# nullmax-vision/SimPB

Hardware: AMD Instinct MI355X
Metric: frames/sec (6-cam sample) + MSDeformAttn HBM GB/s, R50 704x256 @1/2/4/8 GPU (higher is better)
Workload: dtype f32

## Files before the change

include/simpb_hip.h:

```cpp
#ifndef SIMPB_HIP_H
#define SIMPB_HIP_H

#ifdef __cplusplus
extern "C" {
#endif

#define SIMPB_OK 0
#define SIMPB_EINVAL 1
#define SIMPB_ELAUNCH 2

#define SIMPB_RECORD3D_WIDTH 15

int simpb_abi_version(void);

const char* simpb_last_error(void);

#define SIMPB_KERNEL_DAF 1
#define SIMPB_KERNEL_MSDA 2
int simpb_timing_enable(int capacity);
int simpb_timing_read(int kernel_id, float* ms_out, int max_n);
void simpb_timing_reset(void);

int simpb_deformable_aggregation_forward(
    float* output, const float* mc_ms_feat, const int* spatial_shape, const int* scale_start_index,
// ... 276 lines not shown
                           int num_anchors, int num_cams, int num_levels, int num_pts, int num_groups,
                           const unsigned char* cam_valid, void* stream);

int simpb_alloc_project(unsigned char* flag, float* sel_xy, float* depth, const float* anchor,
                        const float* projection_mat, int batch_size, int num_anchors, int num_cams,
                        float img_w, float img_h, float limit_w, float limit_l, float limit_h, void* stream);
int simpb_alloc_project_cams(unsigned char* flag, float* sel_xy, float* depth, const float* anchor,
                             const float* projection_mat, int batch_size, int num_anchors, int num_cams, float img_w,
                             float img_h, float limit_w, float limit_l, float limit_h, const unsigned char* cam_valid,
                             void* stream);

int simpb_alloc_compact(int* count, int* order, const unsigned char* flag, int batch_size, int num_anchors,
                        int num_cams, void* stream);

int simpb_alloc_group_start(int* group_start, int* overflow, const int* count, int batch_size, int num_cams,
                            int capacity, void* stream);

int simpb_alloc_scatter(float* ref_pts2d, float* ref_depth2d, int* q2a, int* is_center, int* a2q, int* query_cam,
                        const int* group_start, const int* count, const int* order, const unsigned char* flag,
                        const float* sel_xy, const float* depth, int batch_size, int num_anchors, int num_cams,
                        int num_query, float img_w, float img_h, void* stream);

int simpb_alloc_static(unsigned char* flag, float* sel_xy, float* depth, int* count, int* order, int* group_start,
                       int* overflow, float* ref_pts2d, float* ref_depth2d, int* q2a, int* is_center, int* a2q,
                       int* query_cam, const float* anchor, const float* projection_mat, int batch_size, int num_anchors,
                       int num_cams, int capacity, float img_w, float img_h, float limit_w, float limit_l, float limit_h,
                       void* stream);
int simpb_alloc_static_cams(unsigned char* flag, float* sel_xy, float* depth, int* count, int* order, int* group_start,
                            int* overflow, float* ref_pts2d, float* ref_depth2d, int* q2a, int* is_center, int* a2q,
                            int* query_cam, const float* anchor, const float* projection_mat, int batch_size,
                            int num_anchors, int num_cams, int capacity, float img_w, float img_h, float limit_w,
                            float limit_l, float limit_h, const unsigned char* cam_valid, void* stream);

int simpb_alloc_ragged(unsigned char* flag, float* sel_xy, float* depth, int* count, int* order, int* group_start,
                       int* overflow, float* ref_pts2d, float* ref_depth2d, int* q2a, int* is_center, int* a2q,
                       int* query_cam, const float* anchor, const float* projection_mat, int batch_size, int num_anchors,
                       int num_cams, int per_stream, float img_w, float img_h, float limit_w, float limit_l, float limit_h,
                       void* stream);
int simpb_alloc_ragged_active(unsigned char* flag, float* sel_xy, float* depth, int* count, int* order, int* group_start,
                              int* overflow, float* ref_pts2d, float* ref_depth2d, int* q2a, int* is_center, int* a2q,
                              int* query_cam, const float* anchor, const float* projection_mat, int batch_size,
                              int num_anchors, int num_cams, int per_stream, float img_w, float img_h, float limit_w,
                              float limit_l, float limit_h, const unsigned char* active, void* stream);
int simpb_alloc_ragged_cams(unsigned char* flag, float* sel_xy, float* depth, int* count, int* order, int* group_start,
                            int* overflow, float* ref_pts2d, float* ref_depth2d, int* q2a, int* is_center, int* a2q,
                            int* query_cam, const float* anchor, const float* projection_mat, int batch_size,
                            int num_anchors, int num_cams, int per_stream, float img_w, float img_h, float limit_w,
                            float limit_l, float limit_h, const unsigned char* active, const unsigned char* cam_valid,
                            void* stream);

int simpb_gather_rows(float* out, const float* src, const int* q2a, int batch_size, int num_anchors,
                      int num_query, int channels, void* stream);

int simpb_aggregate_2d_to_3d(float* out_q, float* out_pos, const float* q3d, const float* pos3d, const float* q2d,
                             const float* pos2d, const float* alpha, const int* a2q, int batch_size,
                             int num_anchors, int num_cams, int num_query, int channels, void* stream);

int simpb_aggregate_2d_to_3d_alpha(float* out_q, float* out_pos, const float* q3d, const float* pos3d, const float* q2d,
                                   const float* pos2d, const float* alpha, const int* a2q, const float* hidden,
                                   int ld_hidden, int hidden_dim, const float* w_alpha, const float* b_alpha,
                                   int batch_size, int num_anchors, int num_cams, int num_query, int channels,
                                   void* stream);

#ifdef __cplusplus
}
#endif
// ... 2 lines not shown
```

simpb_amd/_lib.py:

```python
import ctypes
import os

from .build import LIB

_lib = None

_P = ctypes.c_void_p
_I = ctypes.c_int
_F = ctypes.c_float
_LL = ctypes.c_longlong


class WorldTables(ctypes.Structure):
    _fields_ = [("class_range", _F * 32), ("attr_moving", ctypes.c_ubyte * 32), ("attr_still", ctypes.c_ubyte * 32),
                ("threshold", _F), ("has_threshold", _I), ("num_output", _I)]


SIGNATURES = {
    "simpb_abi_version": ([], _I),
    "simpb_last_error": ([], ctypes.c_char_p),
    "simpb_timing_enable": ([_I], _I),
    "simpb_timing_read": ([_I, _P, _I], _I),
    "simpb_timing_reset": ([], None),
    "simpb_deformable_aggregation_forward": ([_P] * 6 + [_I] * 8 + [_P], _I),
# ... 24 lines not shown
    "simpb_attention_f32_split": ([_P] * 6 + [_I] * 9 + [_F, _P], _I),
    "simpb_attention_split_halfs": ([_P] * 6 + [_I] * 9 + [_P], _I),
    "simpb_mlp_chain_forward": ([_P, _P], _I),
    "simpb_bank_get": ([_P] * 6 + [_I] * 2 + [_F] * 2 + [_P], _I),
    "simpb_bank_update": ([_P] * 10 + [_I] * 5 + [_P], _I),
    "simpb_bank_update_rank": ([_P, _P] + [_I] * 4 + [_P], _I),
    "simpb_bank_update_merge": ([_P] * 13 + [_I, _P] + [_I] * 5 + [_P], _I),
    "simpb_bank_update_merge_active": ([_P] * 13 + [_I, _P] + [_I] * 5 + [_P, _P], _I),
    "simpb_bank_cache": ([_P] * 10 + [_I] * 6 + [_F, _I, _F, _P, _I, _P, _P], _I),
    "simpb_bank_cache_streams": ([_P] * 10 + [_I] * 6 + [_F, _I, _F, _P, _I, _P, _P, _P], _I),
    "simpb_bank_cache_streams_active": ([_P] * 10 + [_I] * 6 + [_F, _I, _F, _P, _I, _P, _P, _P, _P], _I),
    "simpb_decode3d_record": ([_P] * 6 + [_I] * 4 + [_P], _I),
    "simpb_decode2d_record": ([_P] * 6 + [_I] * 4 + [_F] * 4 + [_P], _I),
    "simpb_record2d_compact": ([_P, _LL, _P, _LL, _I, _I, _I, _P], _I),
    "simpb_decode2d_record_ragged": ([_P] * 7 + [_I] * 5 + [_F] * 4 + [_P], _I),
    "simpb_world_record": ([_P] * 5 + [WorldTables, _I, _P], _I),
    "simpb_topk_rows": ([_P, _P, _P, _I, _I, _I, _P], _I),
    "simpb_rowdot_sigmoid": ([_P, _P, _I, _P, _P, _I, _I, _P, _P], _I),
    "simpb_anchor_projection": ([_P] * 4 + [_I] * 2 + [_P], _I),
    "simpb_msda_prep": ([_P, _P, _P, _I, _P, _I, _P, _I, _I, _I, _I, _P, _P], _I),
    "simpb_dfa_points": ([_P] * 7 + [_I] * 5 + [_P], _I),
    "simpb_dfa_weights": ([_P] * 3 + [_I] * 6 + [_P], _I),
    "simpb_dfa_points_cams": ([_P] * 7 + [_I] * 5 + [_P, _P], _I),
    "simpb_dfa_weights_cams": ([_P] * 3 + [_I] * 6 + [_P, _P], _I),
    "simpb_alloc_project_cams": ([_P] * 5 + [_I] * 3 + [_F] * 5 + [_P, _P], _I),
    "simpb_alloc_project": ([_P] * 5 + [_I] * 3 + [_F] * 5 + [_P], _I),
    "simpb_alloc_compact": ([_P] * 3 + [_I] * 3 + [_P], _I),
    "simpb_alloc_group_start": ([_P] * 3 + [_I] * 3 + [_P], _I),
    "simpb_alloc_scatter": ([_P] * 12 + [_I] * 4 + [_F] * 2 + [_P], _I),
    "simpb_alloc_static": ([_P] * 15 + [_I] * 4 + [_F] * 5 + [_P], _I),
    "simpb_alloc_ragged": ([_P] * 15 + [_I] * 4 + [_F] * 5 + [_P], _I),
    "simpb_alloc_ragged_active": ([_P] * 15 + [_I] * 4 + [_F] * 5 + [_P, _P], _I),
    "simpb_alloc_static_cams": ([_P] * 15 + [_I] * 4 + [_F] * 5 + [_P, _P], _I),
    "simpb_alloc_ragged_cams": ([_P] * 15 + [_I] * 4 + [_F] * 5 + [_P, _P, _P], _I),
    "simpb_gather_rows": ([_P] * 3 + [_I] * 4 + [_P], _I),
    "simpb_aggregate_2d_to_3d": ([_P] * 8 + [_I] * 5 + [_P], _I),
    "simpb_aggregate_2d_to_3d_alpha": ([_P] * 9 + [_I, _I, _P, _P] + [_I] * 5 + [_P], _I),
}

ERRORS = {1: "SIMPB_EINVAL (bad pointer/size/layout)", 2: "SIMPB_ELAUNCH (kernel launch failed)"}


def lib():
    global _lib
    if _lib is None:
        if not os.path.exists(LIB):
            raise RuntimeError(
                f"{LIB} is missing: build it with `python -m simpb_amd.build` (hipcc --offload-arch=gfx950). "
                "simpb_amd has no fallback path for its HIP kernels.")
        import torch
        handle = ctypes.CDLL(LIB)
        for name, (argtypes, restype) in SIGNATURES.items():
            fn = getattr(handle, name)
            fn.argtypes = argtypes
            fn.restype = restype
        _lib = handle
    return _lib


def check(status, what):
    if status != 0:
        detail = ""
        if status == 2:
            detail = " - " + (lib().simpb_last_error() or b"").decode()
        raise RuntimeError(f"{what} failed: {ERRORS.get(status, status)}{detail}")
```

simpb_amd/csrc/alloc.hip:

```cpp
#include <hip/hip_runtime.h>
#include "../../include/simpb_hip.h"
#include "store_fence.h"

extern "C" int simpb_check_launch(void);

namespace {

constexpr int kMaxStaticCams = 8;

template <bool MASKED>
__global__ void alloc_project_kernel(unsigned char* __restrict__ flag, float* __restrict__ sel_xy,
                                     float* __restrict__ depth, const float* __restrict__ anchor,
                                     const float* __restrict__ proj, int bs, int A, int cams, float img_w, float img_h,
                                     float lim_w, float lim_l, float lim_h, int* __restrict__ a2q_fill,
                                     const unsigned char* __restrict__ active,
                                     const unsigned char* __restrict__ cam_valid) {
  const int idx = blockIdx.x * blockDim.x + threadIdx.x;
  if (idx >= bs * A * cams) return;
  const int cam = idx % cams;
  const int a = (idx / cams) % A;
  const int b = idx / (cams * A);
  bool off = active && !active[b];
  if (MASKED) off = off || !cam_valid[b * cams + cam];
  if (off) {
    const size_t o = ((size_t)b * cams + cam) * A + a;
    flag[o] = 0;
    sel_xy[2 * o] = 0.f;
    sel_xy[2 * o + 1] = 0.f;
    depth[o] = 0.f;
    if (a2q_fill) a2q_fill[idx] = -1;
    return;
  }
  const float* an = anchor + ((size_t)b * A + a) * 11;
  const float* P = proj + ((size_t)b * cams + cam) * 16;
  const float cx = an[0], cy = an[1], cz = an[2];
  const float sw = fminf(expf(an[3]), lim_w), sl = fminf(expf(an[4]), lim_l), sh = fminf(expf(an[5]), lim_h);
  const float sn = an[6], cs = an[7];

  float xmin = INFINITY, xmax = -INFINITY, ymin = INFINITY, ymax = -INFINITY;
  bool corner_valid = false;
  float ctr_x = 0.f, ctr_y = 0.f, ctr_d = 0.f;
  for (int k = 0; k < 9; ++k) {
    float px, py, pz;
    if (k < 8) {
      const float ox = (((k >> 2) & 1) - 0.5f) * sw, oy = (((k >> 1) & 1) - 0.5f) * sl, oz = ((k & 1) - 0.5f) * sh;
      px = cs * ox - sn * oy + cx;
      py = sn * ox + cs * oy + cy;
      pz = oz + cz;
    } else {
      px = cx; py = cy; pz = cz;
    }
    const float u = P[0] * px + P[1] * py + P[2] * pz + P[3];
    const float v = P[4] * px + P[5] * py + P[6] * pz + P[7];
    const float d = P[8] * px + P[9] * py + P[10] * pz + P[11];
    const float dc = fmaxf(d, 1e-5f);
    const float x = u / dc, y = v / dc;
    const bool inside = 0.f < x && x < img_w && 0.f < y && y < img_h;
    if (k < 8) {
      corner_valid = corner_valid || (d > 0.f && inside);
      xmin = fminf(xmin, x); xmax = fmaxf(xmax, x);
      ymin = fminf(ymin, y); ymax = fmaxf(ymax, y);
    } else {
      ctr_x = x; ctr_y = y; ctr_d = d;
    }
  }
  const bool center_valid = 0.f < ctr_x && ctr_x < img_w && 0.f < ctr_y && ctr_y < img_h;
  float sx = (fminf(fmaxf(xmin, 0.f), img_w) + fminf(fmaxf(xmax, 0.f), img_w)) / 2.f;
  float sy = (fminf(fmaxf(ymin, 0.f), img_h) + fminf(fmaxf(ymax, 0.f), img_h)) / 2.f;
  if (center_valid) { sx = ctr_x; sy = ctr_y; }
  const size_t o = ((size_t)b * cams + cam) * A + a;
  flag[o] = center_valid ? 2 : (corner_valid ? 1 : 0);
  sel_xy[2 * o] = sx;
  sel_xy[2 * o + 1] = sy;
  depth[o] = ctr_d;
  if (a2q_fill) a2q_fill[idx] = -1;
}

__global__ __launch_bounds__(256) void alloc_compact_kernel(int* __restrict__ count, int* __restrict__ order,
                                                            const unsigned char* __restrict__ flag, int A) {
  __shared__ int s_wave[4];
  __shared__ int s_base;
  const int bc = blockIdx.x;
  const unsigned char* f = flag + (size_t)bc * A;
  int* ord = order + (size_t)bc * A;
  const int lane = threadIdx.x & 63, wave = threadIdx.x >> 6;
  if (threadIdx.x == 0) s_base = 0;
  __syncthreads();
  for (int a0 = 0; a0 < A; a0 += 256) {
    const int a = a0 + threadIdx.x;
    const bool on = a < A && f[a] != 0;
    const unsigned long long m = __ballot(on);
    if (lane == 0) s_wave[wave] = __popcll(m);
    __syncthreads();
    int off = s_base;
    for (int w = 0; w < wave; ++w) off += s_wave[w];
    if (on) ord[off + __popcll(m & ((1ull << lane) - 1ull))] = a;
    __syncthreads();
    if (threadIdx.x == 0) s_base += s_wave[0] + s_wave[1] + s_wave[2] + s_wave[3];
    __syncthreads();
  }
  if (threadIdx.x == 0) count[bc] = s_base;
}

__global__ void alloc_scatter_kernel(float* __restrict__ ref_pts2d, float* __restrict__ ref_depth2d,
// ... 124 lines not shown
  is_center[slot] = ctr;
}

__global__ void alloc_group_start_kernel(int* __restrict__ group_start, int* __restrict__ overflow,
                                         const int* __restrict__ count, int bs, int cams, int capacity) {
  if (threadIdx.x != 0 || blockIdx.x != 0) return;
  int acc = 0;
  group_start[0] = 0;
  bool over = false;
  for (int c = 0; c < cams; ++c) {
    int m = 0;
    for (int b = 0; b < bs; ++b) m = max(m, count[b * cams + c]);
    acc += m;
    if (acc > capacity) { over = true; acc = capacity; }
    group_start[c + 1] = acc;
  }
  overflow[0] = over ? 1 : 0;
}

__global__ void fill_int_kernel(int* __restrict__ p, int v, size_t n) {
  const size_t i = (size_t)blockIdx.x * blockDim.x + threadIdx.x;
  if (i < n) p[i] = v;
}

__global__ void gather_rows_kernel(float* __restrict__ out, const float* __restrict__ src,
                                   const int* __restrict__ q2a, int A, int N2, int C4) {
  const int s = blockIdx.x, b = blockIdx.y;
  const int a = q2a[(size_t)b * N2 + s];
  float4* o = reinterpret_cast<float4*>(out) + ((size_t)b * N2 + s) * C4;
  const float4* r = reinterpret_cast<const float4*>(src) + ((size_t)b * A + max(a, 0)) * C4;
  for (int c = threadIdx.x; c < C4; c += blockDim.x) o[c] = a >= 0 ? r[c] : make_float4(0.f, 0.f, 0.f, 0.f);
}

constexpr int kMaxAggCams = 8;
__global__ __launch_bounds__(64) void aggregate_kernel(float* __restrict__ out_q, float* __restrict__ out_pos,
                                                       const float* __restrict__ q3d, const float* __restrict__ pos3d,
                                                       const float* __restrict__ q2d, const float* __restrict__ pos2d,
                                                       const float* __restrict__ alpha, const int* __restrict__ a2q, int A,
                                                       int cams, int N2, int C4, const float* __restrict__ hidden, int ldh,
                                                       int kh, const float* __restrict__ w_alpha,
                                                       const float* __restrict__ b_alpha) {
  const int a = blockIdx.x, b = blockIdx.y;
  const int* slots = a2q + ((size_t)b * A + a) * cams;
  float wgt[kMaxAggCams];
  int slot[kMaxAggCams];
  float div = 0.f;
#pragma unroll
  for (int k = 0; k < kMaxAggCams; ++k) {
    slot[k] = k < cams ? slots[k] : -1;
    wgt[k] = 0.f;
  }
#pragma unroll
  for (int k = 0; k < kMaxAggCams; ++k) {
    const int s = slot[k];
    if (s < 0) continue;
    float w;
    if (hidden) {
      const float* h = hidden + ((size_t)b * N2 + s) * ldh;
      float d = 0.f;
      for (int c = threadIdx.x * 4; c < kh; c += 256) {
        const float4 xv = *reinterpret_cast<const float4*>(h + c);
        const float4 wv = *reinterpret_cast<const float4*>(w_alpha + c);
        d += xv.x * wv.x + xv.y * wv.y + xv.z * wv.z + xv.w * wv.w;
      }
#pragma unroll
      for (int m = 32; m >= 1; m >>= 1) d += __shfl_xor(d, m);
// ... 140 lines not shown
                     out_q, out_pos, q3d, pos3d, q2d, pos2d, alpha, a2q, num_anchors, num_cams, num_query, channels / 4,
                     hidden, ld_hidden, hidden_dim, w_alpha, b_alpha);
  return status();
}

extern "C" int simpb_aggregate_2d_to_3d(float* out_q, float* out_pos, const float* q3d, const float* pos3d,
                                        const float* q2d, const float* pos2d, const float* alpha, const int* a2q,
                                        int batch_size, int num_anchors, int num_cams, int num_query, int channels,
                                        void* stream) {
  if (!alpha) return SIMPB_EINVAL;
  return simpb_aggregate_2d_to_3d_alpha(out_q, out_pos, q3d, pos3d, q2d, pos2d, alpha, a2q, nullptr, 0, 0, nullptr, nullptr,
                                        batch_size, num_anchors, num_cams, num_query, channels, stream);
}

extern "C" int simpb_alloc_static_cams(unsigned char* flag, float* sel_xy, float* depth, int* count, int* order,
                                       int* group_start, int* overflow, float* ref_pts2d, float* ref_depth2d, int* q2a,
                                       int* is_center, int* a2q, int* query_cam, const float* anchor,
                                       const float* projection_mat, int batch_size, int num_anchors, int num_cams, int capacity,
                                       float img_w, float img_h, float limit_w, float limit_l, float limit_h,
                                       const unsigned char* cam_valid, void* stream) {
  if (!flag || !sel_xy || !depth || !count || !order || !group_start || !overflow || !ref_pts2d || !ref_depth2d || !q2a ||
      !is_center || !a2q || !query_cam || !anchor || !projection_mat || batch_size <= 0 || num_anchors <= 0 ||
      num_cams <= 0 || num_cams > kMaxStaticCams || capacity <= 0)
    return SIMPB_EINVAL;
  clear_stale();
  hipStream_t s = static_cast<hipStream_t>(stream);
  launch_project(s, flag, sel_xy, depth, anchor, projection_mat, batch_size, num_anchors, num_cams, img_w, img_h, limit_w,
                 limit_l, limit_h, a2q, nullptr, cam_valid);
  hipLaunchKernelGGL(alloc_compact_kernel, dim3(batch_size * num_cams), dim3(256), 0, s, count, order, flag, num_anchors);
  const int ns = batch_size * capacity;
  hipLaunchKernelGGL(alloc_scatter_kernel, dim3((ns + 255) / 256), dim3(256), 0, s, ref_pts2d, ref_depth2d, q2a, is_center, a2q,
                     query_cam, static_cast<const int*>(nullptr), count, order, flag, sel_xy, depth, batch_size, num_anchors,
                     num_cams, capacity, img_w, img_h, group_start, overflow);
  return status();
}

extern "C" int simpb_alloc_static(unsigned char* flag, float* sel_xy, float* depth, int* count, int* order, int* group_start,
                                  int* overflow, float* ref_pts2d, float* ref_depth2d, int* q2a, int* is_center, int* a2q,
                                  int* query_cam, const float* anchor, const float* projection_mat, int batch_size,
                                  int num_anchors, int num_cams, int capacity, float img_w, float img_h, float limit_w,
                                  float limit_l, float limit_h, void* stream) {
  return simpb_alloc_static_cams(flag, sel_xy, depth, count, order, group_start, overflow, ref_pts2d, ref_depth2d, q2a, is_center,
                                 a2q, query_cam, anchor, projection_mat, batch_size, num_anchors, num_cams, capacity, img_w, img_h,
                                 limit_w, limit_l, limit_h, nullptr, stream);
}

extern "C" int simpb_alloc_ragged_cams(unsigned char* flag, float* sel_xy, float* depth, int* count, int* order,
                                       int* group_start, int* overflow, float* ref_pts2d, float* ref_depth2d, int* q2a,
                                       int* is_center, int* a2q, int* query_cam, const float* anchor,
                                       const float* projection_mat, int batch_size, int num_anchors, int num_cams,
                                       int per_stream, float img_w, float img_h, float limit_w, float limit_l, float limit_h,
                                       const unsigned char* active, const unsigned char* cam_valid, void* stream) {
  if (!flag || !sel_xy || !depth || !count || !order || !group_start || !overflow || !ref_pts2d || !ref_depth2d || !q2a ||
      !is_center || !a2q || !query_cam || !anchor || !projection_mat || batch_size <= 0 || num_anchors <= 0 ||
      num_cams <= 0 || batch_size * num_cams > kMaxRaggedGroups || per_stream <= 0 ||
      (long long)batch_size * per_stream > 0x7fffffffll / 4 || (long long)batch_size * num_anchors > 0x7fffffffll / 4)
    return SIMPB_EINVAL;
  clear_stale();
  hipStream_t s = static_cast<hipStream_t>(stream);
  launch_project(s, flag, sel_xy, depth, anchor, projection_mat, batch_size, num_anchors, num_cams, img_w, img_h, limit_w,
                 limit_l, limit_h, a2q, active, cam_valid);
  hipLaunchKernelGGL(alloc_compact_kernel, dim3(batch_size * num_cams), dim3(256), 0, s, count, order, flag, num_anchors);
  const int ns = batch_size * per_stream;
  hipLaunchKernelGGL(alloc_scatter_ragged_kernel, dim3((ns + 255) / 256), dim3(256), 0, s, ref_pts2d, ref_depth2d, q2a,
                     is_center, a2q, query_cam, count, order, flag, sel_xy, depth, batch_size, num_anchors, num_cams, per_stream,
                     img_w, img_h, group_start, overflow);
// ... 24 lines not shown
```

simpb_amd/plugin/allocation.py:

```python
import ctypes

import torch
import torch.nn as nn

from .. import _lib
from .ops import _ptr, _require_gpu, _stream
from .registry import PLUGIN_LAYERS


from . import routes


class Allocation2D:

    __slots__ = ("q2a", "is_center", "a2q", "query_cam", "query_groups", "num_anchor", "count", "group_start",
                 "overflow", "streams")

    def __init__(self):
        self.streams = 0

    def dense(self):
        if self.streams:
            raise NotImplementedError("a batch of independent streams has no [bs, N2, N3] matrix form")
        bs, n2 = self.q2a.shape
        trans = torch.zeros(bs, n2, self.num_anchor + 1, device=self.q2a.device)
        idx = torch.where(self.q2a >= 0, self.q2a, self.num_anchor).long()
        trans.scatter_(2, idx[..., None], 1.0)
        trans = trans[..., : self.num_anchor].contiguous()
        return trans, trans * self.is_center[..., None].float()


@PLUGIN_LAYERS.register_module()
class DynamicQueryAllocation(nn.Module):
    def __init__(self, with_attn_mask=False, with_project_wh=False, limit_anchor_size=[35, 35, 10],
                 limit_corners_num=[100] * 6):
        super().__init__()
        if with_attn_mask:
            raise NotImplementedError("with_attn_mask is off in the SimPB configs (with_allocate_attn_mask=False)")
        self.with_attn_mask = with_attn_mask
        self.with_project_wh = with_project_wh
        self.limit_anchor_size = limit_anchor_size
        self.limit_corners_num = limit_corners_num
        self.last = None

    def forward(self, anchor3d, metas, dense=True, capacity=None, overflow_out=None, independent=False, active=None,
                cam_valid=None):
        if active is not None and not independent:
            raise ValueError("an activity mask needs the independent-streams layout")
        if independent:
            alloc, ref_pts2d, ref_depth2d = self.allocate_independent(anchor3d, metas, capacity, overflow_out, active,
                                                                      cam_valid)
            if dense:
                raise ValueError("independent streams: index form only (dense=False)")
            return ref_pts2d, ref_depth2d, None, None, None, None, None, None
        alloc, ref_pts2d, ref_depth2d, trans_mask, trans_shape = self.allocate(anchor3d, metas, capacity, overflow_out,
                                                                               cam_valid)
        trans, center = alloc.dense() if dense else (None, None)
        return ref_pts2d, ref_depth2d, trans_mask, trans_shape, trans, center, alloc.query_groups, None

    @staticmethod
    def _check_cam_valid(cam_valid, bs, cams, dev):
        if cam_valid is not None and (not torch.is_tensor(cam_valid) or cam_valid.dtype != torch.uint8
                                      or tuple(cam_valid.shape) != (bs, cams) or cam_valid.device != dev
                                      or not cam_valid.is_contiguous()):
            raise ValueError("camera_valid must be contiguous u8 [bs, cams] on the anchors' device")

    def allocate_independent(self, anchor3d, metas, capacity, overflow_out=None, active=None, cam_valid=None):
        if self.training:
            raise NotImplementedError("training-time corner sampling (allocation.py:85-87) is not on this path")
        if capacity is None:
            raise ValueError("independent streams need a static capacity (slots per stream)")
        _require_gpu(anchor3d)
        lib = _lib.lib()
        anchor3d = anchor3d.contiguous().float()
        proj = metas["projection_mat"].contiguous().float()
        bs, num_anchor = anchor3d.shape[:2]
        cams = proj.shape[1]
        if anchor3d.shape[-1] != 11 or tuple(proj.shape) != (bs, cams, 4, 4):
            raise ValueError("anchor3d must be [bs, N, 11] and projection_mat [bs, cams, 4, 4]")
        wh = metas.get("image_wh_host")
        if wh is None:
            wh = tuple(int(v) for v in metas["image_wh"][0, 0].tolist())
        img_w, img_h = float(wh[0]), float(wh[1])
        dev = anchor3d.device
        if active is not None and (active.dtype != torch.uint8 or active.numel() != bs or active.device != dev
                                   or not active.is_contiguous()):
            raise ValueError("active must be contiguous u8 [bs] on the anchors' device")
        self._check_cam_valid(cam_valid, bs, cams, dev)
        lw, ll, lh = (float(v) for v in self.limit_anchor_size)
        slots = bs * int(capacity)
        flag = torch.empty(bs, cams, num_anchor, dtype=torch.uint8, device=dev)
        sel_xy = torch.empty(bs, cams, num_anchor, 2, device=dev)
        depth = torch.empty(bs, cams, num_anchor, device=dev)
        overflow = overflow_out if overflow_out is not None else torch.empty(1, dtype=torch.int32, device=dev)
        if overflow.dtype != torch.int32 or overflow.numel() != 1 or overflow.device != dev:
            raise ValueError("overflow_out must be one i32 element on the anchors' device")
        out = Allocation2D()
        out.streams = bs
        out.count = torch.empty(bs, cams, dtype=torch.int32, device=dev)
        order = torch.empty(bs, cams, num_anchor, dtype=torch.int32, device=dev)
        out.group_start = torch.empty(bs * cams + 1, dtype=torch.int32, device=dev)
        ref_pts2d = torch.empty(1, slots, 2, device=dev)
        ref_depth2d = torch.empty(1, slots, 1, device=dev)
        out.q2a = torch.empty(1, slots, dtype=torch.int32, device=dev)
        out.is_center = torch.empty(1, slots, dtype=torch.int32, device=dev)
        out.a2q = torch.empty(bs, num_anchor, cams, dtype=torch.int32, device=dev)
        out.query_cam = torch.empty(slots, dtype=torch.int32, device=dev)
        out.query_groups = None
        out.num_anchor = num_anchor
        out.overflow = overflow
        _lib.check(lib.simpb_alloc_ragged_cams(
            _ptr(flag), _ptr(sel_xy), _ptr(depth), _ptr(out.count), _ptr(order), _ptr(out.group_start), _ptr(overflow),
            _ptr(ref_pts2d), _ptr(ref_depth2d), _ptr(out.q2a), _ptr(out.is_center), _ptr(out.a2q), _ptr(out.query_cam),
            _ptr(anchor3d), _ptr(proj), bs, num_anchor, cams, int(capacity), img_w, img_h, lw, ll, lh,
            _ptr(active) if active is not None else None, _ptr(cam_valid) if cam_valid is not None else None, _stream()),
            "simpb_alloc_ragged")
        self.last = out
        return out, ref_pts2d, ref_depth2d

    def allocate(self, anchor3d, metas, capacity=None, overflow_out=None, cam_valid=None):
        if self.training:
            raise NotImplementedError("training-time corner sampling (allocation.py:85-87) is not on this path")
        _require_gpu(anchor3d)
        lib = _lib.lib()
        anchor3d = anchor3d.contiguous().float()
        proj = metas["projection_mat"].contiguous().float()
        bs, num_anchor = anchor3d.shape[:2]
        cams = proj.shape[1]
        if anchor3d.shape[-1] != 11 or tuple(proj.shape) != (bs, cams, 4, 4):
            raise ValueError("anchor3d must be [bs, N, 11] and projection_mat [bs, cams, 4, 4]")
        wh = metas.get("image_wh_host")
        if wh is None:
            wh = tuple(int(v) for v in metas["image_wh"][0, 0].tolist())
        img_w, img_h = float(wh[0]), float(wh[1])
        dev = anchor3d.device
        self._check_cam_valid(cam_valid, bs, cams, dev)
        cv = _ptr(cam_valid) if cam_valid is not None else None
        flag = torch.empty(bs, cams, num_anchor, dtype=torch.uint8, device=dev)
        sel_xy = torch.empty(bs, cams, num_anchor, 2, device=dev)
        depth = torch.empty(bs, cams, num_anchor, device=dev)
        lw, ll, lh = (float(v) for v in self.limit_anchor_size)
        st = _stream()
        count = torch.empty(bs, cams, dtype=torch.int32, device=dev)
        order = torch.empty(bs, cams, num_anchor, dtype=torch.int32, device=dev)
        static = capacity is not None and routes.R.alloc_static_fused and cams <= 8
        if not static:
            _lib.check(lib.simpb_alloc_project_cams(_ptr(flag), _ptr(sel_xy), _ptr(depth), _ptr(anchor3d), _ptr(proj), bs,
                                                    num_anchor, cams, img_w, img_h, lw, ll, lh, cv, st), "simpb_alloc_project")
            _lib.check(lib.simpb_alloc_compact(_ptr(count), _ptr(order), _ptr(flag), bs, num_anchor, cams, st),
                       "simpb_alloc_compact")
        overflow = None
        if capacity is None:
            meta = count.max(dim=0).values.tolist()
            cum = [0]
            for c in meta:
                cum.append(cum[-1] + int(c))
            n2 = cum[-1]
            group_start = torch.tensor(cum, dtype=torch.int32).to(dev, non_blocking=True)
        else:
            cum, n2 = None, int(capacity)
            group_start = torch.empty(cams + 1, dtype=torch.int32, device=dev)
            overflow = overflow_out if overflow_out is not None else torch.empty(1, dtype=torch.int32, device=dev)
            if overflow.dtype != torch.int32 or overflow.numel() != 1 or overflow.device != dev:
                raise ValueError("overflow_out must be one i32 element on the anchors' device")
            if not static:
                _lib.check(lib.simpb_alloc_group_start(_ptr(group_start), _ptr(overflow), _ptr(count), bs, cams, n2, st),
                           "simpb_alloc_group_start")
        ref_pts2d = torch.empty(bs, n2, 2, device=dev)
        ref_depth2d = torch.empty(bs, n2, 1, device=dev)
        out = Allocation2D()
        out.q2a = torch.empty(bs, n2, dtype=torch.int32, device=dev)
        out.is_center = torch.empty(bs, n2, dtype=torch.int32, device=dev)
        out.a2q = torch.empty(bs, num_anchor, cams, dtype=torch.int32, device=dev)
        out.query_cam = torch.empty(n2, dtype=torch.int32, device=dev)
        out.query_groups = [(cum[i], cum[i + 1]) for i in range(cams)] if cum is not None else None
        out.num_anchor = num_anchor
        out.count = count
        out.group_start = group_start
        out.overflow = overflow
        if static:
            _lib.check(lib.simpb_alloc_static_cams(_ptr(flag), _ptr(sel_xy), _ptr(depth), _ptr(count), _ptr(order),
                                                   _ptr(group_start), _ptr(overflow), _ptr(ref_pts2d), _ptr(ref_depth2d),
                                                   _ptr(out.q2a), _ptr(out.is_center), _ptr(out.a2q), _ptr(out.query_cam),
                                                   _ptr(anchor3d), _ptr(proj), bs, num_anchor, cams, n2, img_w, img_h, lw, ll, lh,
                                                   cv, st), "simpb_alloc_static")
        else:
            _lib.check(lib.simpb_alloc_scatter(_ptr(ref_pts2d), _ptr(ref_depth2d), _ptr(out.q2a), _ptr(out.is_center),
                                               _ptr(out.a2q), _ptr(out.query_cam), _ptr(group_start), _ptr(count),
                                               _ptr(order), _ptr(flag), _ptr(sel_xy), _ptr(depth), bs, num_anchor, cams, n2,
                                               img_w, img_h, st), "simpb_alloc_scatter")
        self.last = out
        if capacity is not None:
            return out, ref_pts2d, ref_depth2d, None, None
        trans_mask = (flag != 0).permute(0, 2, 1)
        return out, ref_pts2d, ref_depth2d, trans_mask, count.long()


def gather_rows(src, q2a):
    _require_gpu(src, q2a)
    src = src.contiguous().float()
    bs, num_anchor, c = src.shape
    n2 = q2a.shape[1]
    if q2a.dtype != torch.int32 or not q2a.is_contiguous() or q2a.shape[0] != bs or c % 4:
        raise ValueError("q2a must be contiguous i32 [bs, N2]; channels a multiple of 4")
    out = torch.empty(bs, n2, c, device=src.device)
    if n2:
        _lib.check(_lib.lib().simpb_gather_rows(_ptr(out), _ptr(src), _ptr(q2a), bs, num_anchor, n2, c, _stream()),
                   "simpb_gather_rows")
    return out


def aggregate_2d_to_3d(q3d, pos3d, q2d, pos2d, alpha, a2q, hidden=None, alpha_fc=None):
    _require_gpu(q3d, pos3d, q2d, pos2d, a2q)
# ... 37 lines not shown
```

simpb_amd/plugin/head.py:

```python
from typing import List, Optional

import torch
import torch.nn as nn

from . import training_stubs
from .allocation import gather_rows
from .registry import (ATTENTION, BBOX_CODERS, BBOX_SAMPLERS, FEEDFORWARD_NETWORK, HEADS, LOSSES, NORM_LAYERS,
                       PLUGIN_LAYERS, POSITIONAL_ENCODING, TRANSFORMER_LAYER_SEQUENCE, build_from_cfg)
from . import dense, routes
from .layers import BaseModule, fused_graph_attention

__all__ = ["SimPBHead"]


@HEADS.register_module()
class SimPBHead(BaseModule):
    def __init__(self, instance_bank: dict, anchor_encoder: dict, graph_model: dict, norm_layer: dict, ffn: dict,
                 deformable_model: dict, num_cams: int = 6, num_decoder: int = 6, num_single_frame_decoder: int = -1,
                 temp_graph_model: dict = None, loss_cls: dict = None, loss_reg: dict = None, decoder: dict = None,
                 sampler: dict = None, reg_weights: List = None, operation_order: Optional[List[str]] = None,
                 cls_threshold_to_reg: float = -1, dn_loss_weight: float = 5.0, decouple_attn: bool = True,
                 init_cfg: dict = None, enable2d=False, enable3d=True, embed_dims=256, num_levels=4, num_anchor=900,
                 encoder2d=None, share_encoder2d=False, anchor_encoder2d=None, positional_encoding=None,
                 qg_self_attn=None, qg_cross_attn=None, refine_layer2d=None, refine_layer3d=None,
# ... 215 lines not shown
                raise ValueError("metas['camera_valid'] must be a contiguous u8 [bs, cams] tensor on the device")
        if split:
            if "time_interval" not in metas or self.static_capacity is None:
                raise ValueError("forward_split needs metas['time_interval'] (f32 [bs]) and a static capacity")
            instance_feature, anchor = self.instance_bank.learned(batch_size)
            temp_instance_feature = temp_anchor = None
            time_interval = metas["time_interval"]
        else:
            instance_feature, anchor, temp_instance_feature, temp_anchor, time_interval = self.instance_bank.get(
                batch_size, metas, dn_metas=None)
        if temp_anchor is not None and anchor.is_cuda:
            both = self.anchor_encoder.forward(torch.cat([anchor, temp_anchor], dim=1))
            anchor_embed = dense.report(self.anchor_encoder, both[:, : anchor.shape[1]])
            temp_anchor_embed = dense.report(self.anchor_encoder, both[:, anchor.shape[1]:])
        else:
            anchor_embed = self.anchor_encoder(anchor)
            temp_anchor_embed = self.anchor_encoder(temp_anchor) if temp_anchor is not None else None

        quality, prediction, classification = [], [], []
        prediction2d, classification2d, prediction_alpha2d, prediction_depth2d = [], [], [], []
        ref_pts2d_list, ref_trans_shape_list, ref_trans_matrix_list, ref_query_groups_list = [], [], [], []
        alloc_list = []
        cap = self.static_capacity
        temp_attn_instance = instance_feature
        pre_values = feature_maps[3] if len(feature_maps) > 3 else None
        encoder2d_dict, feature_maps = self.prepare2d(feature_maps, metas)
        cam_embeds = self._camera_embeddings(metas, batch_size)
        alloc = None
        self._m_live = None
        last = len(self.operation_order) - 1
        n_refine2d = sum(op == "refine2d" and layer is not None for op, layer in zip(self.operation_order, self.layers))
        pending_norm = None
        overflow = hold = sticky = None
        if cap is not None:
            n_alloc = sum(op == "allocation" for op in self.operation_order)
            chain = metas.get("overflow_chain")
            sticky = None
            if split:
                hb, sticky = metas["overflow_split"]
                if hb.dtype != torch.int32 or hb.numel() != n_alloc + 1 or sticky.dtype != torch.int32 or sticky.numel() != 1:
                    raise ValueError("overflow_split: (i32 [allocation layers + 1], i32 [1])")
                overflow = hb[:n_alloc]
                overflow.zero_()
                hold = hb
            elif chain is not None:
                flags, row = chain
                if flags.dtype != torch.int32 or flags.dim() != 2 or flags.shape[1] != n_alloc or not flags.is_contiguous():
                    raise ValueError("overflow_chain: (contiguous i32 [rows, allocation layers] tensor, row)")
                overflow = flags[row]
                overflow.zero_()
                hold = flags.view(-1)
            else:
                overflow = hold = torch.zeros(n_alloc, dtype=torch.int32, device=anchor.device)

        for i, op in enumerate(self.operation_order):
            layer = self.layers[i]
            if layer is None:
                continue
            elif op == "norm":
                nxt = self.operation_order[i + 1] if i < last else None
                if (instance_feature.is_cuda and routes.R.dense and routes.R.norm_in_refine and routes.R.chain_rows4
                        and nxt in ("refine2d", "refine3d") and self.layers[i + 1] is not None
                        and torch.is_tensor(instance_feature) and abs(layer.eps - 1e-5) < 1e-12):
                    pending_norm = layer
                elif instance_feature.is_cuda and routes.R.dense:
                    instance_feature = dense.layernorm(instance_feature, layer, m_live=self._m_live)
                else:
                    instance_feature = layer(instance_feature)
            elif op == "ffn":
                instance_feature = layer(instance_feature, m_live=self._m_live)
            elif op == "allocation":
                assert self.instance_status == "3d"
                k = len(ref_pts2d_list)
                if self.independent_streams and batch_size > 1 and cap is None:
                    raise ValueError("independent_streams needs a static capacity (the flat slot array has a fixed size)")
                ragged = self.independent_streams and batch_size > 1
                anchor2d, ref_depth2d, ref_trans_mask, ref_trans_shape, _, _, ref_query_groups, _ = layer(
                    anchor, metas, dense=False, capacity=cap,
                    overflow_out=overflow[k:k + 1] if overflow is not None else None, independent=ragged, active=active,
                    cam_valid=camera_valid)
                alloc = layer.last
                if ragged:
                    groups = batch_size * self.num_cams
                    self._m_live = alloc.group_start[groups: groups + 1]
                    instance_feature = instance_feature.reshape(1, -1, instance_feature.shape[-1])
                elif cap is not None and batch_size == 1 and alloc.group_start is not None:
                    self._m_live = alloc.group_start[self.num_cams: self.num_cams + 1]
                instance_feature = gather_rows(instance_feature, alloc.q2a)
                anchor_embed2d = (self.anchor_encoder2d(anchor2d, m_live=self._m_live) if self._m_live is not None
                                  else self.anchor_encoder2d(anchor2d))
                ref_pts2d_list.append(anchor2d[..., :2])
                self.instance_status = "2d"
            elif op == "aggregation":
                assert self.instance_status == "2d"
                instance_feature, anchor_embed, anchor = layer(
                    query2d=instance_feature, query_pos2d=anchor_embed2d, anchor2d=anchor2d,
                    query3d=temp_attn_instance, query_pos3d=anchor_embed, anchor3d=anchor,
                    allocation=alloc, attn_mask=None, graph_model=self.graph_model, m_live=self._m_live)
                self.instance_status = "3d"
                self._m_live = None
            elif op == "qg_self_attn":
                instance_feature = self.graph_model2d(i, query=instance_feature, value=instance_feature,
                                                      query_pos=anchor_embed2d, query_groups=ref_query_groups,
                                                      query_cam=alloc.query_cam, group_start=alloc.group_start)
            elif op == "qg_cross_attn":
                enc = encoder2d_dict
                if pre_values is not None and i in pre_values:
                    enc = dict(encoder2d_dict, value=pre_values[i], value_is_projected=True)
                instance_feature = layer(query=instance_feature, query_pos=anchor_embed2d,
                                         reference_points=anchor2d.unsqueeze(2), query_groups=ref_query_groups,
                                         query_cam=alloc.query_cam, m_live=self._m_live,
                                         keep_parts=routes.R.dense and self._next_is_ffn(i), **enc)
            elif op == "refine2d":
                kw = dict(m_live=self._m_live) if self._m_live is not None else {}
                if lean and len(prediction2d) < n_refine2d - 1:
                    if pending_norm is not None:
                        instance_feature, pending_norm = dense.report(pending_norm, layer.norm_alone(instance_feature, pending_norm, **kw)), None
                    anchor2d = cls2d = depth2d = alpha2d = None
                else:
                    if pending_norm is not None:
                        kw["norm"] = pending_norm
# ... 101 lines not shown
```

simpb_amd/plugin/routes.py:

```python
import contextlib

DEFAULTS = dict(
    dense=True,
    gemm_split_fp16=True,
    attention_split_fp16=True,
    chain_rows4=True,
    chain_transposed=False,
    split_value_proj=True,
    fused_decode=True,
    fused_bank=True,
    bank_cache_per_stream=True,
    parallel_branches=False,
    conv1x1_kernel=True,
    conv3x3_kernel=True,
    stem_epilogue_kernel=True,
    stem_kernel=True,
    fpn_grouped_out=True,
    alloc_static_fused=True,
    msda_linear=True,
    norm_in_refine=True,
    fused_dfa=True,
    dfa_f16_tokens=True,
    lean_tokens=True,
    lean_refine2d=True,
    lean_glue=True,
)


class _Routes:
    __slots__ = tuple(DEFAULTS) + ("_open",)

    def __init__(self):
        object.__setattr__(self, "_open", False)
        for k, v in DEFAULTS.items():
            object.__setattr__(self, k, v)

    def __setattr__(self, name, value):
        if not self._open:
            raise AttributeError(f"routes.R.{name} is read-only: use `with routes.override({name}=...)` (tests / tools only)")
        if name not in DEFAULTS:
            raise AttributeError(f"no route named {name!r}")
        object.__setattr__(self, name, bool(value))

    def __repr__(self):
        return "Routes(" + ", ".join(f"{k}={getattr(self, k)}" for k in DEFAULTS) + ")"


R = _Routes()


@contextlib.contextmanager
# ... 17 lines not shown
```

Baseline: 421.9.

## Fuse static allocation into two launches with compaction, row gather and flag clearing

```diff
diff --git a/include/simpb_hip.h b/include/simpb_hip.h
--- a/include/simpb_hip.h
+++ b/include/simpb_hip.h
@@ -332,6 +332,13 @@
                             int num_anchors, int num_cams, int capacity, float img_w, float img_h, float limit_w,
                             float limit_l, float limit_h, const unsigned char* cam_valid, void* stream);
 
+int simpb_alloc_static_rows(unsigned char* flag, float* sel_xy, float* depth, int* count, int* order, int* group_start,
+                            int* overflow, float* ref_pts2d, float* ref_depth2d, int* q2a, int* is_center, int* a2q,
+                            int* query_cam, float* rows_out, const float* rows_src, const float* anchor,
+                            const float* projection_mat, int* clear_flags, int batch_size, int num_anchors, int num_cams,
+                            int capacity, int channels, int num_clear, float img_w, float img_h, float limit_w,
+                            float limit_l, float limit_h, const unsigned char* cam_valid, void* stream);
+
 int simpb_alloc_ragged(unsigned char* flag, float* sel_xy, float* depth, int* count, int* order, int* group_start,
                        int* overflow, float* ref_pts2d, float* ref_depth2d, int* q2a, int* is_center, int* a2q,
                        int* query_cam, const float* anchor, const float* projection_mat, int batch_size, int num_anchors,
diff --git a/simpb_amd/_lib.py b/simpb_amd/_lib.py
--- a/simpb_amd/_lib.py
+++ b/simpb_amd/_lib.py
@@ -80,6 +80,7 @@
     "simpb_alloc_ragged": ([_P] * 15 + [_I] * 4 + [_F] * 5 + [_P], _I),
     "simpb_alloc_ragged_active": ([_P] * 15 + [_I] * 4 + [_F] * 5 + [_P, _P], _I),
     "simpb_alloc_static_cams": ([_P] * 15 + [_I] * 4 + [_F] * 5 + [_P, _P], _I),
+    "simpb_alloc_static_rows": ([_P] * 18 + [_I] * 6 + [_F] * 5 + [_P, _P], _I),
     "simpb_alloc_ragged_cams": ([_P] * 15 + [_I] * 4 + [_F] * 5 + [_P, _P, _P], _I),
     "simpb_gather_rows": ([_P] * 3 + [_I] * 4 + [_P], _I),
     "simpb_aggregate_2d_to_3d": ([_P] * 8 + [_I] * 5 + [_P], _I),
diff --git a/simpb_amd/csrc/alloc.hip b/simpb_amd/csrc/alloc.hip
--- a/simpb_amd/csrc/alloc.hip
+++ b/simpb_amd/csrc/alloc.hip
@@ -7,6 +7,50 @@
 namespace {
 
 constexpr int kMaxStaticCams = 8;
+
+__device__ __forceinline__ unsigned char project_anchor(const float* an, const float* P, float img_w, float img_h,
+                                                        float lim_w, float lim_l, float lim_h, float& sel_x, float& sel_y,
+                                                        float& ctr_depth) {
+  const float cx = an[0], cy = an[1], cz = an[2];
+  const float sw = fminf(expf(an[3]), lim_w), sl = fminf(expf(an[4]), lim_l), sh = fminf(expf(an[5]), lim_h);
+  const float sn = an[6], cs = an[7];
+
+  float xmin = INFINITY, xmax = -INFINITY, ymin = INFINITY, ymax = -INFINITY;
+  bool corner_valid = false;
+  float ctr_x = 0.f, ctr_y = 0.f, ctr_d = 0.f;
+  for (int k = 0; k < 9; ++k) {
+    float px, py, pz;
+    if (k < 8) {
+      const float ox = (((k >> 2) & 1) - 0.5f) * sw, oy = (((k >> 1) & 1) - 0.5f) * sl, oz = ((k & 1) - 0.5f) * sh;
+      px = cs * ox - sn * oy + cx;
+      py = sn * ox + cs * oy + cy;
+      pz = oz + cz;
+    } else {
+      px = cx; py = cy; pz = cz;
+    }
+    const float u = P[0] * px + P[1] * py + P[2] * pz + P[3];
+    const float v = P[4] * px + P[5] * py + P[6] * pz + P[7];
+    const float d = P[8] * px + P[9] * py + P[10] * pz + P[11];
+    const float dc = fmaxf(d, 1e-5f);
+    const float x = u / dc, y = v / dc;
+    const bool inside = 0.f < x && x < img_w && 0.f < y && y < img_h;
+    if (k < 8) {
+      corner_valid = corner_valid || (d > 0.f && inside);
+      xmin = fminf(xmin, x); xmax = fmaxf(xmax, x);
+      ymin = fminf(ymin, y); ymax = fmaxf(ymax, y);
+    } else {
+      ctr_x = x; ctr_y = y; ctr_d = d;
+    }
+  }
+  const bool center_valid = 0.f < ctr_x && ctr_x < img_w && 0.f < ctr_y && ctr_y < img_h;
+  float sx = (fminf(fmaxf(xmin, 0.f), img_w) + fminf(fmaxf(xmax, 0.f), img_w)) / 2.f;
+  float sy = (fminf(fmaxf(ymin, 0.f), img_h) + fminf(fmaxf(ymax, 0.f), img_h)) / 2.f;
+  if (center_valid) { sx = ctr_x; sy = ctr_y; }
+  sel_x = sx;
+  sel_y = sy;
+  ctr_depth = ctr_d;
+  return center_valid ? 2 : (corner_valid ? 1 : 0);
+}
 
 template <bool MASKED>
 __global__ void alloc_project_kernel(unsigned char* __restrict__ flag, float* __restrict__ sel_xy,
@@ -31,45 +75,11 @@
     if (a2q_fill) a2q_fill[idx] = -1;
     return;
   }
-  const float* an = anchor + ((size_t)b * A + a) * 11;
-  const float* P = proj + ((size_t)b * cams + cam) * 16;
-  const float cx = an[0], cy = an[1], cz = an[2];
-  const float sw = fminf(expf(an[3]), lim_w), sl = fminf(expf(an[4]), lim_l), sh = fminf(expf(an[5]), lim_h);
-  const float sn = an[6], cs = an[7];
-
-  float xmin = INFINITY, xmax = -INFINITY, ymin = INFINITY, ymax = -INFINITY;
-  bool corner_valid = false;
-  float ctr_x = 0.f, ctr_y = 0.f, ctr_d = 0.f;
-  for (int k = 0; k < 9; ++k) {
-    float px, py, pz;
-    if (k < 8) {
-      const float ox = (((k >> 2) & 1) - 0.5f) * sw, oy = (((k >> 1) & 1) - 0.5f) * sl, oz = ((k & 1) - 0.5f) * sh;
-      px = cs * ox - sn * oy + cx;
-      py = sn * ox + cs * oy + cy;
-      pz = oz + cz;
-    } else {
-      px = cx; py = cy; pz = cz;
-    }
-    const float u = P[0] * px + P[1] * py + P[2] * pz + P[3];
-    const float v = P[4] * px + P[5] * py + P[6] * pz + P[7];
-    const float d = P[8] * px + P[9] * py + P[10] * pz + P[11];
-    const float dc = fmaxf(d, 1e-5f);
-    const float x = u / dc, y = v / dc;
-    const bool inside = 0.f < x && x < img_w && 0.f < y && y < img_h;
-    if (k < 8) {
-      corner_valid = corner_valid || (d > 0.f && inside);
-      xmin = fminf(xmin, x); xmax = fmaxf(xmax, x);
-      ymin = fminf(ymin, y); ymax = fmaxf(ymax, y);
-    } else {
-      ctr_x = x; ctr_y = y; ctr_d = d;
-    }
-  }
-  const bool center_valid = 0.f < ctr_x && ctr_x < img_w && 0.f < ctr_y && ctr_y < img_h;
-  float sx = (fminf(fmaxf(xmin, 0.f), img_w) + fminf(fmaxf(xmax, 0.f), img_w)) / 2.f;
-  float sy = (fminf(fmaxf(ymin, 0.f), img_h) + fminf(fmaxf(ymax, 0.f), img_h)) / 2.f;
-  if (center_valid) { sx = ctr_x; sy = ctr_y; }
+  float sx, sy, ctr_d;
+  const unsigned char f = project_anchor(anchor + ((size_t)b * A + a) * 11, proj + ((size_t)b * cams + cam) * 16, img_w, img_h,
+                                         lim_w, lim_l, lim_h, sx, sy, ctr_d);
   const size_t o = ((size_t)b * cams + cam) * A + a;
-  flag[o] = center_valid ? 2 : (corner_valid ? 1 : 0);
+  flag[o] = f;
   sel_xy[2 * o] = sx;
   sel_xy[2 * o + 1] = sy;
   depth[o] = ctr_d;
@@ -260,6 +270,142 @@
   for (int c = threadIdx.x; c < C4; c += blockDim.x) o[c] = a >= 0 ? r[c] : make_float4(0.f, 0.f, 0.f, 0.f);
 }
 
+constexpr int kProjectThreads = 1024;
+template <bool MASKED>
+__global__ __launch_bounds__(kProjectThreads) void alloc_project_compact_kernel(
+    unsigned char* __restrict__ flag, float* __restrict__ sel_xy, float* __restrict__ depth, int* __restrict__ count,
+    int* __restrict__ order, int* __restrict__ a2q_fill, const float* __restrict__ anchor, const float* __restrict__ proj, int A,
+    int cams, float img_w, float img_h, float lim_w, float lim_l, float lim_h, const unsigned char* __restrict__ cam_valid,
+    int* __restrict__ clear, int n_clear) {
+  constexpr int kWaves = kProjectThreads / 64;
+  __shared__ int s_wave[kWaves];
+  const int bc = blockIdx.x;
+  const int b = bc / cams, cam = bc - b * cams;
+  const int lane = threadIdx.x & 63, wave = threadIdx.x >> 6;
+  bool off = false;
+  if (MASKED) off = !cam_valid[bc];
+  float P[12];
+#pragma unroll
+  for (int i = 0; i < 12; ++i) P[i] = off ? 0.f : proj[(size_t)bc * 16 + i];
+  int base = 0;
+  for (int a0 = 0; a0 < A; a0 += kProjectThreads) {
+    if (a0 > 0) {
+      simpb::stores_retired();
+      __syncthreads();
+    }
+    const int a = a0 + threadIdx.x;
+    const bool live = a < A;
+    float an[8];
+#pragma unroll
+    for (int i = 0; i < 8; ++i) an[i] = (live && !off) ? anchor[((size_t)b * A + a) * 11 + i] : 0.f;
+    simpb::loads_retired();
+    float sx, sy, ctr_d;
+    int f = project_anchor(an, P, img_w, img_h, lim_w, lim_l, lim_h, sx, sy, ctr_d);
+    if (off) { f = 0; sx = 0.f; sy = 0.f; ctr_d = 0.f; }
+    simpb::pin(f); simpb::pin(sx); simpb::pin(sy); simpb::pin(ctr_d);
+    const bool on = live && f != 0;
+    const unsigned long long m = __ballot(on);
+    if (lane == 0) s_wave[wave] = __popcll(m);
+    __syncthreads();
+    int at = base + __popcll(m & ((1ull << lane) - 1ull));
+#pragma unroll
+    for (int w = 0; w < kWaves; ++w) {
+      const int n = s_wave[w];
+      if (w < wave) at += n;
+      base += n;
+    }
+    simpb::pin(at);
+    if (live) {
+      const size_t o = (size_t)bc * A + a;
+      flag[o] = (unsigned char)f;
+      sel_xy[2 * o] = sx;
+      sel_xy[2 * o + 1] = sy;
+      depth[o] = ctr_d;
+      a2q_fill[((size_t)b * A + a) * cams + cam] = -1;
+      if (on) order[(size_t)bc * A + at] = a;
+    }
+  }
+  if (threadIdx.x == 0) count[bc] = base;
+  if (bc == 0 && clear)
+    for (int i = threadIdx.x; i < n_clear; i += kProjectThreads) clear[i] = 0;
+}
+
+__global__ __launch_bounds__(64) void alloc_scatter_rows_kernel(
+    float* __restrict__ ref_pts2d, float* __restrict__ ref_depth2d, int* __restrict__ q2a, int* __restrict__ is_center,
+    int* __restrict__ a2q, int* __restrict__ query_cam, const int* __restrict__ count, const int* __restrict__ order,
+    const unsigned char* __restrict__ flag, const float* __restrict__ sel_xy, const float* __restrict__ depth, int bs, int A,
+    int cams, int N2, float img_w, float img_h, int* __restrict__ group_start_out, int* __restrict__ overflow_out,
+    float* __restrict__ rows_out, const float* __restrict__ rows_src, int C4) {
+  const int slot = blockIdx.x, b = blockIdx.y;
+  const int idx = b * N2 + slot;
+  int cam = 0, g_lo = 0, g_end = 0;
+  int gs[kMaxStaticCams];
+  bool over = false;
+  {
+    int acc = 0;
+    bool found = false;
+#pragma unroll
+    for (int c = 0; c < kMaxStaticCams; ++c) {
+      gs[c] = acc;
+      if (c < cams) {
+        int m = 0;
+        for (int bb = 0; bb < bs; ++bb) m = max(m, count[bb * cams + c]);
+        const int lo = acc;
+        acc += m;
+        if (acc > N2) { over = true; acc = N2; }
+        if (!found && (slot < acc || c == cams - 1)) { cam = c; g_lo = lo; found = true; }
+        gs[c] = acc;
+      }
+    }
+    g_end = acc;
+  }
+  const int rank = slot - g_lo;
+  const bool in_set = slot < g_end;
+  const int bc = b * cams + cam;
+  float x = 0.f, y = 0.f, d = 0.f;
+  int a = -1, ctr = 0;
+  if (in_set && rank < count[bc]) {
+    a = order[(size_t)bc * A + rank];
+    const size_t o = (size_t)bc * A + a;
+    x = sel_xy[2 * o] / img_w;
+    y = sel_xy[2 * o + 1] / img_h;
+    d = fabsf(depth[o]);
+    ctr = flag[o] == 2;
+  }
+  const float4* r = reinterpret_cast<const float4*>(rows_src) + ((size_t)b * A + max(a, 0)) * C4;
+  float4* o4 = reinterpret_cast<float4*>(rows_out) + (size_t)idx * C4;
+  int c = threadIdx.x;
+  float4 v = make_float4(0.f, 0.f, 0.f, 0.f);
+  if (a >= 0 && c < C4) v = r[c];
+  simpb::pin(x); simpb::pin(y); simpb::pin(d); simpb::pin(a); simpb::pin(ctr);
+  simpb::pin(v.x); simpb::pin(v.y); simpb::pin(v.z); simpb::pin(v.w);
+  simpb::loads_retired();
+  if (threadIdx.x == 0) {
+    if (idx == 0) {
+      group_start_out[0] = 0;
+#pragma unroll
+      for (int k = 0; k < kMaxStaticCams; ++k)
+        if (k < cams) group_start_out[k + 1] = gs[k];
+      overflow_out[0] = over ? 1 : 0;
+    }
+    if (b == 0) query_cam[slot] = in_set ? cam : -1;
+    if (a >= 0) a2q[((size_t)b * A + a) * cams + cam] = slot;
+    ref_pts2d[2 * (size_t)idx] = x;
+    ref_pts2d[2 * (size_t)idx + 1] = y;
+    ref_depth2d[idx] = d;
+    q2a[idx] = a;
+    is_center[idx] = ctr;
+  }
+  if (c < C4) o4[c] = v;
+  for (c += 64; c < C4; c += 64) {
+    simpb::stores_retired();
+    v = a >= 0 ? r[c] : make_float4(0.f, 0.f, 0.f, 0.f);
+    simpb::pin(v.x); simpb::pin(v.y); simpb::pin(v.z); simpb::pin(v.w);
+    simpb::loads_retired();
+    o4[c] = v;
+  }
+}
+
 constexpr int kMaxAggCams = 8;
 __global__ __launch_bounds__(64) void aggregate_kernel(float* __restrict__ out_q, float* __restrict__ out_pos,
                                                        const float* __restrict__ q3d, const float* __restrict__ pos3d,
@@ -466,6 +612,37 @@
   hipLaunchKernelGGL(alloc_scatter_kernel, dim3((ns + 255) / 256), dim3(256), 0, s, ref_pts2d, ref_depth2d, q2a, is_center, a2q,
                      query_cam, static_cast<const int*>(nullptr), count, order, flag, sel_xy, depth, batch_size, num_anchors,
                      num_cams, capacity, img_w, img_h, group_start, overflow);
+  return status();
+}
+
+extern "C" int simpb_alloc_static_rows(unsigned char* flag, float* sel_xy, float* depth, int* count, int* order,
+                                       int* group_start, int* overflow, float* ref_pts2d, float* ref_depth2d, int* q2a,
+                                       int* is_center, int* a2q, int* query_cam, float* rows_out, const float* rows_src,
+                                       const float* anchor, const float* projection_mat, int* clear_flags, int batch_size,
+                                       int num_anchors, int num_cams, int capacity, int channels, int num_clear, float img_w,
+                                       float img_h, float limit_w, float limit_l, float limit_h,
+                                       const unsigned char* cam_valid, void* stream) {
+  if (!flag || !sel_xy || !depth || !count || !order || !group_start || !overflow || !ref_pts2d || !ref_depth2d || !q2a ||
+      !is_center || !a2q || !query_cam || !rows_out || !rows_src || !anchor || !projection_mat || batch_size <= 0 ||
+      batch_size > 65535 || num_anchors <= 0 || num_cams <= 0 || num_cams > kMaxStaticCams || capacity <= 0 || channels <= 0 ||
+      channels % 4 != 0 || num_clear < 0 || (num_clear > 0 && !clear_flags) ||
+      (long long)batch_size * num_anchors * num_cams > 0x7fffffffll || (long long)batch_size * capacity > 0x7fffffffll ||
+      ((reinterpret_cast<size_t>(rows_out) | reinterpret_cast<size_t>(rows_src)) & 15))
+    return SIMPB_EINVAL;
+  clear_stale();
+  hipStream_t s = static_cast<hipStream_t>(stream);
+  int* clear = num_clear > 0 ? clear_flags : nullptr;
+  if (cam_valid)
+    hipLaunchKernelGGL(alloc_project_compact_kernel<true>, dim3(batch_size * num_cams), dim3(kProjectThreads), 0, s, flag, sel_xy, depth,
+                       count, order, a2q, anchor, projection_mat, num_anchors, num_cams, img_w, img_h, limit_w, limit_l, limit_h,
+                       cam_valid, clear, num_clear);
+  else
+    hipLaunchKernelGGL(alloc_project_compact_kernel<false>, dim3(batch_size * num_cams), dim3(kProjectThreads), 0, s, flag, sel_xy, depth,
+                       count, order, a2q, anchor, projection_mat, num_anchors, num_cams, img_w, img_h, limit_w, limit_l, limit_h,
+                       static_cast<const unsigned char*>(nullptr), clear, num_clear);
+  hipLaunchKernelGGL(alloc_scatter_rows_kernel, dim3(capacity, batch_size), dim3(64), 0, s, ref_pts2d, ref_depth2d, q2a,
+                     is_center, a2q, query_cam, count, order, flag, sel_xy, depth, batch_size, num_anchors, num_cams, capacity,
+                     img_w, img_h, group_start, overflow, rows_out, rows_src, channels / 4);
   return status();
 }
 
diff --git a/simpb_amd/plugin/allocation.py b/simpb_amd/plugin/allocation.py
--- a/simpb_amd/plugin/allocation.py
+++ b/simpb_amd/plugin/allocation.py
@@ -14,10 +14,11 @@
 class Allocation2D:
 
     __slots__ = ("q2a", "is_center", "a2q", "query_cam", "query_groups", "num_anchor", "count", "group_start",
-                 "overflow", "streams")
+                 "overflow", "streams", "rows")
 
     def __init__(self):
         self.streams = 0
+        self.rows = None
 
     def dense(self):
         if self.streams:
@@ -43,8 +44,15 @@
         self.limit_corners_num = limit_corners_num
         self.last = None
 
+    @staticmethod
+    def two_launches(capacity, cams, independent=False):
+        return (capacity is not None and not independent and cams <= 8 and routes.R.alloc_static_fused
+                and routes.R.alloc_two_launches)
+
     def forward(self, anchor3d, metas, dense=True, capacity=None, overflow_out=None, independent=False, active=None,
-                cam_valid=None):
+                cam_valid=None, rows=None, clear=None):
+        if independent and (rows is not None or clear is not None):
+            raise ValueError("independent streams: no rows / clear (the four-launch form)")
         if active is not None and not independent:
             raise ValueError("an activity mask needs the independent-streams layout")
         if independent:
@@ -54,7 +62,7 @@
                 raise ValueError("independent streams: index form only (dense=False)")
             return ref_pts2d, ref_depth2d, None, None, None, None, None, None
         alloc, ref_pts2d, ref_depth2d, trans_mask, trans_shape = self.allocate(anchor3d, metas, capacity, overflow_out,
-                                                                               cam_valid)
+                                                                               cam_valid, rows=rows, clear=clear)
         trans, center = alloc.dense() if dense else (None, None)
         return ref_pts2d, ref_depth2d, trans_mask, trans_shape, trans, center, alloc.query_groups, None
 
@@ -118,7 +126,7 @@
         self.last = out
         return out, ref_pts2d, ref_depth2d
 
-    def allocate(self, anchor3d, metas, capacity=None, overflow_out=None, cam_valid=None):
+    def allocate(self, anchor3d, metas, capacity=None, overflow_out=None, cam_valid=None, rows=None, clear=None):
         if self.training:
             raise NotImplementedError("training-time corner sampling (allocation.py:85-87) is not on this path")
         _require_gpu(anchor3d)
@@ -144,6 +152,17 @@
         count = torch.empty(bs, cams, dtype=torch.int32, device=dev)
         order = torch.empty(bs, cams, num_anchor, dtype=torch.int32, device=dev)
         static = capacity is not None and routes.R.alloc_static_fused and cams <= 8
+        two = rows is not None and self.two_launches(capacity, cams)
+        if clear is not None and not two:
+            raise ValueError("clear: only the two-launch route (a static capacity and `rows`) clears flags")
+        if two:
+            _require_gpu(rows)
+            rows = rows.contiguous().float()
+            if rows.dim() != 3 or tuple(rows.shape[:2]) != (bs, num_anchor) or rows.shape[2] % 4 or rows.device != dev:
+                raise ValueError("rows must be f32 [bs, num_anchor, C] on the anchors' device, C a multiple of 4")
+            if clear is not None and (clear.dtype != torch.int32 or clear.dim() != 1 or not clear.is_contiguous()
+                                      or clear.device != dev):
+                raise ValueError("clear must be a contiguous i32 vector on the anchors' device")
         if not static:
             _lib.check(lib.simpb_alloc_project_cams(_ptr(flag), _ptr(sel_xy), _ptr(depth), _ptr(anchor3d), _ptr(proj), bs,
                                                     num_anchor, cams, img_w, img_h, lw, ll, lh, cv, st), "simpb_alloc_project")
@@ -178,7 +197,15 @@
         out.count = count
         out.group_start = group_start
         out.overflow = overflow
-        if static:
+        if two:
+            out.rows = torch.empty(bs, n2, rows.shape[2], device=dev)
+            _lib.check(lib.simpb_alloc_static_rows(
+                _ptr(flag), _ptr(sel_xy), _ptr(depth), _ptr(count), _ptr(order), _ptr(group_start), _ptr(overflow),
+                _ptr(ref_pts2d), _ptr(ref_depth2d), _ptr(out.q2a), _ptr(out.is_center), _ptr(out.a2q), _ptr(out.query_cam),
+                _ptr(out.rows), _ptr(rows), _ptr(anchor3d), _ptr(proj), _ptr(clear) if clear is not None else None, bs,
+                num_anchor, cams, n2, rows.shape[2], clear.numel() if clear is not None else 0, img_w, img_h, lw, ll, lh, cv,
+                st), "simpb_alloc_static_rows")
+        elif static:
             _lib.check(lib.simpb_alloc_static_cams(_ptr(flag), _ptr(sel_xy), _ptr(depth), _ptr(count), _ptr(order),
                                                    _ptr(group_start), _ptr(overflow), _ptr(ref_pts2d), _ptr(ref_depth2d),
                                                    _ptr(out.q2a), _ptr(out.is_center), _ptr(out.a2q), _ptr(out.query_cam),
diff --git a/simpb_amd/plugin/head.py b/simpb_amd/plugin/head.py
--- a/simpb_amd/plugin/head.py
+++ b/simpb_amd/plugin/head.py
@@ -271,8 +271,16 @@
         n_refine2d = sum(op == "refine2d" and layer is not None for op, layer in zip(self.operation_order, self.layers))
         pending_norm = None
         overflow = hold = sticky = None
+        clear_in_alloc = False
         if cap is not None:
             n_alloc = sum(op == "allocation" for op in self.operation_order)
+            live = [(op, layer) for op, layer in zip(self.operation_order, self.layers) if layer is not None]
+            ops_live = [op for op, _ in live]
+            first_alloc = ops_live.index("allocation") if "allocation" in ops_live else -1
+            alloc_layer = live[first_alloc][1] if first_alloc >= 0 else None
+            clear_in_alloc = (first_alloc >= 0 and "refine3d" not in ops_live[:first_alloc] and anchor.is_cuda
+                              and hasattr(alloc_layer, "two_launches")
+                              and alloc_layer.two_launches(cap, self.num_cams, self.independent_streams and batch_size > 1))
             chain = metas.get("overflow_chain")
             sticky = None
             if split:
@@ -280,17 +288,20 @@
                 if hb.dtype != torch.int32 or hb.numel() != n_alloc + 1 or sticky.dtype != torch.int32 or sticky.numel() != 1:
                     raise ValueError("overflow_split: (i32 [allocation layers + 1], i32 [1])")
                 overflow = hb[:n_alloc]
-                overflow.zero_()
+                if not clear_in_alloc:
+                    overflow.zero_()
                 hold = hb
             elif chain is not None:
                 flags, row = chain
                 if flags.dtype != torch.int32 or flags.dim() != 2 or flags.shape[1] != n_alloc or not flags.is_contiguous():
                     raise ValueError("overflow_chain: (contiguous i32 [rows, allocation layers] tensor, row)")
                 overflow = flags[row]
-                overflow.zero_()
+                if not clear_in_alloc:
+                    overflow.zero_()
                 hold = flags.view(-1)
             else:
-                overflow = hold = torch.zeros(n_alloc, dtype=torch.int32, device=anchor.device)
+                overflow = hold = (torch.empty if clear_in_alloc else torch.zeros)(n_alloc, dtype=torch.int32,
+                                                                                  device=anchor.device)
 
         for i, op in enumerate(self.operation_order):
             layer = self.layers[i]
@@ -314,10 +325,16 @@
                 if self.independent_streams and batch_size > 1 and cap is None:
                     raise ValueError("independent_streams needs a static capacity (the flat slot array has a fixed size)")
                 ragged = self.independent_streams and batch_size > 1
+                kw = {}
+                if cap is not None and anchor.is_cuda and hasattr(layer, "two_launches") and layer.two_launches(
+                        cap, self.num_cams, ragged):
+                    kw = dict(rows=instance_feature, clear=overflow if clear_in_alloc and k == 0 else None)
+                elif clear_in_alloc and k == 0:
+                    raise RuntimeError("the frame's overflow flags were left to an allocation that does not clear them")
                 anchor2d, ref_depth2d, ref_trans_mask, ref_trans_shape, _, _, ref_query_groups, _ = layer(
                     anchor, metas, dense=False, capacity=cap,
                     overflow_out=overflow[k:k + 1] if overflow is not None else None, independent=ragged, active=active,
-                    cam_valid=camera_valid)
+                    cam_valid=camera_valid, **kw)
                 alloc = layer.last
                 if ragged:
                     groups = batch_size * self.num_cams
@@ -325,7 +342,7 @@
                     instance_feature = instance_feature.reshape(1, -1, instance_feature.shape[-1])
                 elif cap is not None and batch_size == 1 and alloc.group_start is not None:
                     self._m_live = alloc.group_start[self.num_cams: self.num_cams + 1]
-                instance_feature = gather_rows(instance_feature, alloc.q2a)
+                instance_feature = alloc.rows if alloc.rows is not None else gather_rows(instance_feature, alloc.q2a)
                 anchor_embed2d = (self.anchor_encoder2d(anchor2d, m_live=self._m_live) if self._m_live is not None
                                   else self.anchor_encoder2d(anchor2d))
                 ref_pts2d_list.append(anchor2d[..., :2])
diff --git a/simpb_amd/plugin/routes.py b/simpb_amd/plugin/routes.py
--- a/simpb_amd/plugin/routes.py
+++ b/simpb_amd/plugin/routes.py
@@ -17,6 +17,7 @@
     stem_kernel=True,
     fpn_grouped_out=True,
     alloc_static_fused=True,
+    alloc_two_launches=True,
     msda_linear=True,
     norm_in_refine=True,
     fused_dfa=True,
```

Result: slower. 415.9 (-1.4%).
